# CityU-AIM-Group/SCAN

Measured on AMD Instinct MI355X. Metric: train images/sec (whole node), VGG16 C2F 1024x2048, higher is better.
Workload: dtype f32 (fp32 storage, fp32 multiply, fp32 accumulate -- the reference's arithmetic; the convolutions run it on the bf16 matrix cores as bf16x6: every fp32 operand cut into 3 bf16 pieces = all 24 significand bits, 6 bf16 MFMAs per product)

## Files before the change

### scan_amd/csrc/capi.cpp

```cpp
#include <stdarg.h>
#include <stdio.h>
#include <string.h>

#include "../../include/scan_hip.h"

static thread_local char g_err[512] = "";

extern "C" void scan_set_error(const char* fmt, ...) {
  va_list ap;
  va_start(ap, fmt);
  vsnprintf(g_err, sizeof(g_err), fmt, ap);
  va_end(ap);
}

extern "C" const char* scan_last_error(void) { return g_err; }
extern "C" int scan_abi_version(void) { return 1; }

extern int g_scan_conv_bn256;
extern int g_scan_conv_v2;
extern int g_scan_conv_wg1024;
extern int g_scan_conv_w8;
extern int g_scan_conv_tpb3;
extern int g_scan_conv_bn64_th16;
extern int g_scan_conv_glds;
extern int g_scan_conv1x1;
extern int g_scan_conv_wino;
extern int g_scan_wgrad_v6;
extern int g_scan_wgrad_prio;
extern int g_scan_wgrad_tile;
extern int g_scan_wgrad_wgs;
extern int g_scan_wgrad_wino;
extern int g_scan_gconv_mfma;
extern int g_scan_dbscan_bf16x3;
extern int g_scan_reduce_blocks;

struct Knob {
  const char* key;
  int* slot;
  int dflt;
};
static Knob* knob_table(int* count) {
  static Knob knobs[] = {
      {"conv_bn256", &g_scan_conv_bn256, 0},   {"conv_v2", &g_scan_conv_v2, 0},         {"conv_wg1024", &g_scan_conv_wg1024, 0},
      {"conv_w8", &g_scan_conv_w8, 0},         {"conv_tpb3", &g_scan_conv_tpb3, 0},     {"conv_bn64_th16", &g_scan_conv_bn64_th16, 0},
      {"conv_glds", &g_scan_conv_glds, 0},     {"wgrad_v6", &g_scan_wgrad_v6, 0},       {"wgrad_prio", &g_scan_wgrad_prio, 0},
      {"wgrad_tile", &g_scan_wgrad_tile, 0},   {"wgrad_wgs", &g_scan_wgrad_wgs, 0},     {"gconv_mfma", &g_scan_gconv_mfma, 0},
      {"dbscan_bf16x3", &g_scan_dbscan_bf16x3, 0}, {"reduce_blocks", &g_scan_reduce_blocks, 0}, {"conv1x1", &g_scan_conv1x1, 0},
      {"conv_wino", &g_scan_conv_wino, 0},     {"wgrad_wino", &g_scan_wgrad_wino, 0},
  };
  static bool init = false;
  if (!init) {
    for (auto& k : knobs) k.dflt = *k.slot;
    init = true;
  }
  *count = (int)(sizeof(knobs) / sizeof(knobs[0]));
  return knobs;
}
static Knob* find_knob(const char* key) {
  int n = 0;
  Knob* t = knob_table(&n);
  if (key == nullptr) return nullptr;
  for (int i = 0; i < n; ++i)
    if (strcmp(key, t[i].key) == 0) return &t[i];
  return nullptr;
}

extern "C" int scan_tune(const char* key, int value) {
  Knob* k = find_knob(key);
  if (k == nullptr) return SCAN_TUNE_UNKNOWN;
  const int old = *k->slot;
  *k->slot = value;
  return old;
}

extern "C" int scan_tune_get(const char* key) {
  const Knob* k = find_knob(key);
  return k == nullptr ? SCAN_TUNE_UNKNOWN : *k->slot;
}

extern "C" int scan_tune_default(const char* key) {
  const Knob* k = find_knob(key);
  return k == nullptr ? SCAN_TUNE_UNKNOWN : k->dflt;
}

extern "C" const char* scan_tune_key(int index) {
  int n = 0;
  const Knob* t = knob_table(&n);
  return (index >= 0 && index < n) ? t[index].key : nullptr;
}
```

### scan_amd/csrc/conv_fwd.hip

```cpp
#include "conv_split.h"

#define V2_TW 16
#ifndef SCAN_CONV_MID
#define SCAN_CONV_MID 0
#endif
#ifndef SCAN_CONV_PFA
#define SCAN_CONV_PFA 1
#endif
#define V2_CK 32

struct TileTab2 {
  int tile_off[SCAN_MAX_LEVELS + 1];
  int tiles_x[SCAN_MAX_LEVELS];
  int tiles_y[SCAN_MAX_LEVELS];
};

__device__ __forceinline__ int swz(int idx) { return (idx >> 1) & 2; }
__device__ __forceinline__ int wsw(int t, int r) { return ((t >> 1) & 2) ^ (r & 1); }

template <int K>
__device__ __forceinline__ const __bf16* pick_plane(const __bf16* w0, const __bf16* w1, const __bf16* w2) {
  if constexpr (K == 0)
    return w0;
  else if constexpr (K == 1)
    return w1;
  else
    return w2;
}
template <int I, int NT, int PL, int NPL>
__device__ __forceinline__ const __bf16* slot_plane(int tid, const __bf16* w0, const __bf16* w1, const __bf16* w2) {
  constexpr int lo = (NT * I) / PL, hi = (NT * I + NT - 1) / PL;
  constexpr int lo_c = lo < NPL ? lo : NPL - 1, hi_c = hi < NPL ? hi : NPL - 1;
  static_assert(hi - lo <= 1, "a thread's slot spans at most two planes");
  if constexpr (lo_c == hi_c)
    return pick_plane<lo_c>(w0, w1, w2);
  else
    return (tid + NT * I) / PL == lo ? pick_plane<lo_c>(w0, w1, w2) : pick_plane<hi_c>(w0, w1, w2);
}
template <int NT, int PL, int NPL>
__device__ __forceinline__ const __bf16* slot_plane_i(int i, int tid, const __bf16* w0, const __bf16* w1, const __bf16* w2) {
  return i == 0   ? slot_plane<0, NT, PL, NPL>(tid, w0, w1, w2)
         : i == 1 ? slot_plane<1, NT, PL, NPL>(tid, w0, w1, w2)
         : i == 2 ? slot_plane<2, NT, PL, NPL>(tid, w0, w1, w2)
         : i == 3 ? slot_plane<3, NT, PL, NPL>(tid, w0, w1, w2)
         : i == 4 ? slot_plane<4, NT, PL, NPL>(tid, w0, w1, w2)
                  : slot_plane<5, NT, PL, NPL>(tid, w0, w1, w2);
}

template <int NP, int TM>
__device__ __forceinline__ void mma_pieces(const bf16x8 (&w)[NP], const bf16x8 (&p)[NP][TM], f32x4v (&acc)[TM]) {
#pragma unroll
  for (int s = NP - 1; s >= 0; --s)
#pragma unroll
    for (int i = 0; i <= s; ++i)
#pragma unroll
      for (int tm = 0; tm < TM; ++tm) acc[tm] = __builtin_amdgcn_mfma_f32_16x16x32_bf16(w[i], p[s - i][tm], acc[tm], 0, 0, 0);
}

template <int NP, int BN, int TH, int NT, int KS, int TPB = 1, bool GL = false, bool WINO = false>
__global__ __launch_bounds__(NT, NT == 1024 ? 4 : 2) void conv_split_kernel(
    const float* __restrict__ src, scan_pyramid_t d, int Cs, const __bf16* __restrict__ w0, const __bf16* __restrict__ w1,
    const __bf16* __restrict__ w2, int Csw, const float* __restrict__ bias, const float* __restrict__ mask,
    float* __restrict__ dst, int Nout, int Ns, int relu, TileTab2 tt, int n_tiles, scan_pyramid_t sd, int map,
    double* __restrict__ gn_ws) {
  constexpr int HALO = KS / 2, NTAPS = KS * KS;
  constexpr int PH = TH + 2 * HALO;
  constexpr int PWK = WINO ? 32 : V2_TW + 2 * HALO;
  constexpr int NPATCH = PH * PWK;
  constexpr int WTAPS = WINO ? 12 : NTAPS;
  constexpr int WAVES = NT / 64;
  constexpr int WN_WAVES = BN >= 128 ? 2 : 1;
  constexpr int WM_WAVES = WAVES / WN_WAVES;
  constexpr int TM = TH / WM_WAVES;
  constexpr int TN = BN / (16 * WN_WAVES);
  constexpr int TMW = WINO ? TM / 2 : TM;
  constexpr int ASLOTS = WINO ? (PH * 64 + NT - 1) / NT : (NPATCH * 8 + NT - 1) / NT;
  constexpr int AK = WINO ? 4 : 1;
  constexpr int BSLOTS = BN * 4 * NP;
  constexpr int BSEG = (BSLOTS + NT - 1) / NT;
  constexpr int NGRP = WTAPS / TPB;
  static_assert(NP == 2 || NP == 3, "two or three pieces per operand");
  static_assert(TM * WM_WAVES == TH && (TM % 2) == 0, "tile rows must split evenly (and pair up for the fused pool)");
  static_assert(NTAPS % TPB == 0, "taps per barrier must divide the tap count");
  static_assert(BSLOTS % 64 == 0, "a wave's 64 weight segments lie in one plane (and past the end only as a whole wave)");
  static_assert(!WINO || (GL && KS == 3 && TPB == 1 && NP == 3 && TM % 2 == 0), "Winograd: three pieces, 3x3, LDS-DMA weights");

  extern __shared__ __align__(16) unsigned char smem_raw[];
  __bf16* As = reinterpret_cast<__bf16*>(smem_raw);
  __bf16* Bs = As + NP * NPATCH * 32;

  const int tid = threadIdx.x, lane = tid & 63, wid = tid >> 6;
  const int bid = xcd_remap(blockIdx.x, gridDim.x);
  const int n_tile = bid % n_tiles;
  const int tile = bid / n_tiles;
  int lvl = 0;
#pragma unroll
  for (int i = 1; i < SCAN_MAX_LEVELS; ++i)
    if (i < d.n_levels && tile >= tt.tile_off[i]) lvl = i;
  const int H = d.h[lvl], W = d.w[lvl];
  int t = tile - tt.tile_off[lvl];
  const int per_img = tt.tiles_x[lvl] * tt.tiles_y[lvl];
  const int img = t / per_img;
  t -= img * per_img;
  const int ty0 = (t / tt.tiles_x[lvl]) * TH, tx0 = (t % tt.tiles_x[lvl]) * V2_TW;
  const int64_t rowbase = d.row_off[lvl] + (int64_t)img * H * W;
  const int n0 = n_tile * BN;
  const int nchunks = (Cs + V2_CK - 1) / V2_CK;

  constexpr unsigned BAD = 0x80000000u;
  unsigned voff[ASLOTS];
  unsigned vok = 0;
  const int c_tail = Cs - (nchunks - 1) * V2_CK;
  const bool tail_bad = 4 * (tid & 7) >= c_tail;
  __amdgpu_buffer_rsrc_t a_src;
  {
    const bool mapped = KS == 1 && map != 0;
    const int Hs = mapped ? sd.h[lvl] : H, Ws = mapped ? sd.w[lvl] : W;
    int64_t base_row;
    if (!mapped)
      base_row = rowbase + (int64_t)(ty0 - HALO) * W + (tx0 - HALO);
    else if (map == 1)
      base_row = sd.row_off[lvl] + ((int64_t)img * Hs + 2 * ty0) * Ws + 2 * tx0;
    else
      base_row = sd.row_off[lvl] + ((int64_t)img * Hs + (ty0 >> 1)) * Ws + (tx0 >> 1);
    a_src = uniform_rsrc_b(src + base_row * Cs, 0x7ffffff0);
    if constexpr (WINO) {
#pragma unroll
      for (int i = 0; i < ASLOTS; ++i) {
        const int slot = tid + NT * i;
        const int c4 = slot & 7, t = (slot >> 3) & 7, py = slot >> 6;
        voff[i] = (unsigned)(((py * W + 2 * t) * Cs + 4 * c4) * 4);
#pragma unroll
        for (int k = 0; k < 4; ++k) {
          const int y = ty0 - HALO + py, x = tx0 - HALO + 2 * t + k;
          if ((slot < PH * 64) && y >= 0 && y < H && x >= 0 && x < W) vok |= 1u << (4 * i + k);
        }
      }
    } else {
#pragma unroll
      for (int i = 0; i < ASLOTS; ++i) {
        const int slot = tid + NT * i;
        const int q = slot >> 3, c4 = slot & 7;
        const int py = q / PWK, px = q - py * PWK;
        const int y = ty0 - HALO + py, x = tx0 - HALO + px;
        bool ok = (slot < NPATCH * 8) && y >= 0 && y < H && x >= 0 && x < W;
        int pix = py * W + px;
        if (mapped) {
          if (map == 1) {
            ok = ok && 2 * y < Hs && 2 * x < Ws;
            pix = 2 * py * Ws + 2 * px;
          } else {
            ok = ok && ((y | x) & 1) == 0 && (y >> 1) < Hs && (x >> 1) < Ws;
            pix = (py >> 1) * Ws + (px >> 1);
          }
        }
        voff[i] = ok ? (unsigned)((pix * Cs + 4 * c4) * 4) : BAD;
      }
    }
  }
  float4 ra[ASLOTS][AK];
  auto load_a = [&](int cc) {
    const int soff = cc * (V2_CK * 4);
    const bool kill = tail_bad && cc == nchunks - 1;
#pragma unroll
    for (int i = 0; i < ASLOTS; ++i)
#pragma unroll
      for (int k = 0; k < AK; ++k) {
        const unsigned off = !WINO ? voff[i] : ((vok >> (4 * i + k)) & 1) ? voff[i] + (unsigned)(k * Cs * 4) : BAD;
        ra[i][k] = __builtin_bit_cast(float4, __builtin_amdgcn_raw_buffer_load_b128(a_src, (int)(kill ? BAD : off), soff, 0));
      }
  };
  auto store_a = [&]() {
    if constexpr (WINO) {
#pragma unroll
      for (int i = 0; i < ASLOTS; ++i) {
        const int slot = tid + NT * i;
        if (slot < PH * 64) {
          const int c4 = slot & 7, t = (slot >> 3) & 7, py = slot >> 6;
          const float4 d0 = ra[i][0], d1 = ra[i][1], d2 = ra[i][2], d3 = ra[i][3];
          const float4 u[4] = {make_float4(d0.x - d2.x, d0.y - d2.y, d0.z - d2.z, d0.w - d2.w),
                               make_float4(d1.x + d2.x, d1.y + d2.y, d1.z + d2.z, d1.w + d2.w),
                               make_float4(d2.x - d1.x, d2.y - d1.y, d2.z - d1.z, d2.w - d1.w),
                               make_float4(d1.x - d3.x, d1.y - d3.y, d1.z - d3.z, d1.w - d3.w)};
          const int sl = (((c4 >> 1) ^ wsw(t, py)) << 3) + ((c4 & 1) << 2);
#pragma unroll
          for (int j = 0; j < 4; ++j) {
            bf16x4 pc[NP];
            split4_np<NP>(u[j], pc);
            const int off = (py * PWK + j * 8 + t) * 32 + sl;
#pragma unroll
            for (int p = 0; p < NP; ++p) *reinterpret_cast<bf16x4*>(As + p * NPATCH * 32 + off) = pc[p];
          }
        }
      }
      return;
    }
#pragma unroll
    for (int i = 0; i < ASLOTS; ++i) {
      const int slot = tid + NT * i;
      if (slot < NPATCH * 8) {
        const int q = slot >> 3, c4 = slot & 7;
        const int px = q % PWK;
        bf16x4 pc[NP];
        split4_np<NP>(ra[i][0], pc);
        const int off = q * 32 + (((c4 >> 1) ^ swz(px)) << 3) + ((c4 & 1) << 2);
#pragma unroll
        for (int p = 0; p < NP; ++p) *reinterpret_cast<bf16x4*>(As + p * NPATCH * 32 + off) = pc[p];
      }
    }
  };
  uint4 rb[TPB][BSEG];
  auto load_b = [&](int cc, int grp) {
#pragma unroll
    for (int tt = 0; tt < TPB; ++tt) {
      const int tap = grp * TPB + tt;
#pragma unroll
      for (int i = 0; i < BSEG; ++i) {
        const int slot = tid + NT * i;
        const int plane = slot / (BN * 4);
        const int rem = slot - plane * BN * 4;
        const int row = rem >> 2, seg = rem & 3;
        const int o = n0 + row, c = cc * V2_CK + 8 * seg;
        const __bf16* base = slot_plane_i<NT, BN * 4, NP>(i, tid, w0, w1, w2);
        rb[tt][i] = (slot < BSLOTS && o < Nout && c < Csw)
                        ? *reinterpret_cast<const uint4*>(base + ((int64_t)o * NTAPS + tap) * Csw + c)
                        : make_uint4(0u, 0u, 0u, 0u);
      }
    }
  };
  auto store_b = [&](int buf) {
#pragma unroll
    for (int tt = 0; tt < TPB; ++tt) {
#pragma unroll
      for (int i = 0; i < BSEG; ++i) {
        const int slot = tid + NT * i;
        const int plane = slot / (BN * 4);
        const int rem = slot - plane * BN * 4;
        const int row = rem >> 2, seg = rem & 3;
        if (slot < BSLOTS)
          *reinterpret_cast<uint4*>(Bs + (((buf * TPB + tt) * NP + plane) * BN + row) * 32 + ((seg ^ swz(row)) << 3)) = rb[tt][i];
      }
    }
  };

  static_assert(!GL || BSEG <= 6, "the LDS-DMA path keeps at most six descriptors");
  unsigned boff[BSEG];
#pragma unroll
  for (int i = 0; i < BSEG; ++i) {
    const int slot = tid + NT * i;
    const int plane = slot / (BN * 4);
    const int rem = slot - plane * BN * 4;
    const int row = rem >> 2, seg = (rem & 3) ^ swz(row);
    boff[i] = (unsigned)((((n0 + row) * WTAPS) * Csw + 8 * seg) * 2);
  }
  const int plane_bytes = Nout * WTAPS * Csw * 2;
  auto plane_rsrc = [&](int i) { return uniform_rsrc_b(slot_plane_i<NT, BN * 4, NP>(i, tid, w0, w1, w2), plane_bytes); };
  const __amdgpu_buffer_rsrc_t b_src0 = plane_rsrc(0), b_src1 = plane_rsrc(1), b_src2 = plane_rsrc(2),
                               b_src3 = plane_rsrc(3), b_src4 = plane_rsrc(4), b_src5 = plane_rsrc(5);
  auto issue_b = [&](int cc, int grp, int buf) {
#pragma unroll
    for (int tt = 0; tt < TPB; ++tt) {
      const int tap = grp * TPB + tt;
      const int soff = (tap * Csw + cc * V2_CK) * 2;
#pragma unroll
      for (int i = 0; i < BSEG; ++i) {
        const int slot = tid + NT * i;
        if (BSEG * NT != BSLOTS && slot - lane >= BSLOTS) continue;
        const int plane = slot / (BN * 4);
        const int rem = slot - plane * BN * 4;
        __bf16* dst_l = Bs + (((buf * TPB + tt) * NP + plane) * BN) * 32 + (rem - lane) * 8;
        __builtin_amdgcn_raw_ptr_buffer_load_lds(
            i == 0 ? b_src0 : i == 1 ? b_src1 : i == 2 ? b_src2 : i == 3 ? b_src3 : i == 4 ? b_src4 : b_src5, (lds_ptr_t)dst_l,
            16, (int)boff[i], soff, 0, 0);
      }
    }
  };

  const int wm = wid / WN_WAVES, wn = wid % WN_WAVES;
  const int lr = lane & 15, kg = lane >> 4;
  const int w_row0 = wn * 16 * TN + lr;
  const int w_off = w_row0 * 32 + ((kg ^ swz(w_row0)) << 3);

  f32x4v acc[TN][TM];
#pragma unroll
  for (int b = 0; b < TN; ++b)
#pragma unroll
    for (int a = 0; a < TM; ++a) acc[b][a] = f32x4v{0.f, 0.f, 0.f, 0.f};
  f32x4v wacc[WINO ? 4 : 1][WINO ? TN : 1][TMW];
#pragma unroll
  for (int j = 0; j < (WINO ? 4 : 1); ++j)
#pragma unroll
    for (int b = 0; b < (WINO ? TN : 1); ++b)
#pragma unroll
      for (int a = 0; a < TMW; ++a) wacc[j][b][a] = f32x4v{0.f, 0.f, 0.f, 0.f};

  auto patch_off = [&](int tap) {
    const int ky = tap / KS, kx = tap - KS * ky;
    const int pxs = lr + kx;
    return ((wm * TM + ky) * PWK + pxs) * 32 + ((kg ^ swz(pxs)) << 3);
  };
  auto read_patch = [&](int tap, bf16x8 (&pf)[NP][TM]) {
    const int p_off = patch_off(tap);
#pragma unroll
    for (int p = 0; p < NP; ++p)
#pragma unroll
      for (int tm = 0; tm < TM; ++tm)
        pf[p][tm] = *reinterpret_cast<const bf16x8*>(As + p * NPATCH * 32 + p_off + tm * PWK * 32);
  };
  auto read_w = [&](const __bf16* bt, int tn, bf16x8 (&wf)[NP]) {
#pragma unroll
    for (int p = 0; p < NP; ++p) wf[p] = *reinterpret_cast<const bf16x8*>(bt + p * BN * 32 + tn * 16 * 32);
  };
  auto taps_mma = [&](int grp, int buf, auto&& mid) {
#pragma unroll
    for (int tt = 0; tt < TPB; ++tt) {
      const int tap = grp * TPB + tt;
      const __bf16* bt = Bs + ((buf * TPB + tt) * NP) * BN * 32 + w_off;
      bf16x8 pf[NP][TM];
      read_patch(tap, pf);
#pragma unroll
      for (int tn = 0; tn < TN; ++tn) {
        bf16x8 wf[NP];
        read_w(bt, tn, wf);
        mma_pieces<NP, TM>(wf, pf, acc[tn]);
#ifdef SCAN_EXP_MID_STAGGER
        if (tt == 0 && tn == ((wid >= WAVES / 2 && TN >= 8) ? SCAN_EXP_MID_STAGGER : SCAN_CONV_MID)) {
#else
        if (tt == 0 && tn == SCAN_CONV_MID) {
#endif
          __builtin_amdgcn_sched_barrier(0);
          mid();
          __builtin_amdgcn_sched_barrier(0);
        }
      }
    }
  };
  auto no_mid = []() {};

  constexpr bool PFA = GL && NT == 512 && TPB == 1 && NP == 2 && SCAN_CONV_PFA;
  bf16x8 npf[NP][TM];
  auto taps_mma_pf = [&](int grp, int buf, auto&& mid) {
    if constexpr (PFA) {
      const __bf16* bt = Bs + (buf * NP) * BN * 32 + w_off;
      if (grp == 0) read_patch(0, npf);
#pragma unroll
      for (int tn = 0; tn < TN - 1; ++tn) {
        bf16x8 wf[NP];
        read_w(bt, tn, wf);
        mma_pieces<NP, TM>(wf, npf, acc[tn]);
        if (tn == SCAN_CONV_MID) {
          __builtin_amdgcn_sched_barrier(0);
          mid();
          __builtin_amdgcn_sched_barrier(0);
        }
      }
      {
        constexpr int tn = TN - 1;
        bf16x8 wf[NP];
        read_w(bt, tn, wf);
        const bool more = grp < NGRP - 1;
        const int p_off = patch_off(more ? grp + 1 : grp);
#pragma unroll
        for (int tm = 0; tm < TM; ++tm) {
          acc[tn][tm] = __builtin_amdgcn_mfma_f32_16x16x32_bf16(wf[0], npf[1][tm], acc[tn][tm], 0, 0, 0);
          acc[tn][tm] = __builtin_amdgcn_mfma_f32_16x16x32_bf16(wf[1], npf[0][tm], acc[tn][tm], 0, 0, 0);
          acc[tn][tm] = __builtin_amdgcn_mfma_f32_16x16x32_bf16(wf[0], npf[0][tm], acc[tn][tm], 0, 0, 0);
          npf[0][tm] = *reinterpret_cast<const bf16x8*>(As + p_off + tm * PWK * 32);
          npf[1][tm] = *reinterpret_cast<const bf16x8*>(As + NPATCH * 32 + p_off + tm * PWK * 32);
        }
      }
    }
  };

  auto wino_mma = [&](int j, int ky, int buf, f32x4v (&aj)[WINO ? TN : 1][TMW], auto&& mid) {
    const __bf16* bt = Bs + (buf * NP) * BN * 32 + w_off;
    const int prow = wm * TM + (lr >> 3) + ky, t = lr & 7;
    const int p_off = (prow * PWK + j * 8 + t) * 32 + ((kg ^ wsw(t, prow)) << 3);
    bf16x8 pf[NP][TMW];
#pragma unroll
    for (int p = 0; p < NP; ++p)
#pragma unroll
      for (int tm = 0; tm < TMW; ++tm)
        pf[p][tm] = *reinterpret_cast<const bf16x8*>(As + p * NPATCH * 32 + p_off + tm * 2 * PWK * 32);
#pragma unroll
    for (int tn = 0; tn < TN; ++tn) {
      bf16x8 wf[NP];
      read_w(bt, tn, wf);
      mma_pieces<NP, TMW>(wf, pf, aj[tn]);
      if (tn == (SCAN_CONV_MID >= 0 ? SCAN_CONV_MID : 0)) {
        __builtin_amdgcn_sched_barrier(0);
        mid();
        __builtin_amdgcn_sched_barrier(0);
      }
    }
  };

  load_a(0);
  if constexpr (WINO) {
    issue_b(0, 0, 0);
    for (int cc = 0; cc < nchunks; ++cc) {
      __syncthreads();
      store_a();
      auto comp = [&](int j, f32x4v (&aj)[WINO ? TN : 1][TMW]) {
#pragma unroll 1
        for (int ky = 0; ky < 3; ++ky) {
          const int grp = j * 3 + ky, buf = grp & 1;
          asm volatile("s_waitcnt vmcnt(0)" ::: "memory");
          __syncthreads();
          auto feed = [&]() {
            if (grp < NGRP - 1)
              issue_b(cc, grp + 1, buf ^ 1);
            else if (cc + 1 < nchunks)
              issue_b(cc + 1, 0, buf ^ 1);
            if (grp == NGRP - 2 && cc + 1 < nchunks) load_a(cc + 1);
          };
          wino_mma(j, ky, buf, aj, feed);
        }
      };
      comp(0, wacc[0]);
      comp(1, wacc[WINO ? 1 : 0]);
      comp(2, wacc[WINO ? 2 : 0]);
      comp(3, wacc[WINO ? 3 : 0]);
    }
  } else if constexpr (GL) {
    issue_b(0, 0, 0);
    for (int cc = 0; cc < nchunks; ++cc) {
      __syncthreads();
#ifdef SCAN_EXP_FWD_NOFEED
      if (cc == 0 || !(SCAN_EXP_FWD_NOFEED & 2))
#endif
      store_a();
      if (NGRP == 1 && cc + 1 < nchunks) load_a(cc + 1);
#pragma unroll 1
      for (int grp = 0; grp < NGRP; ++grp) {
        const int buf = (cc * NGRP + grp) & 1;
        asm volatile("s_waitcnt vmcnt(0)" ::: "memory");
        __syncthreads();
        auto feed = [&]() {
#ifdef SCAN_EXP_FWD_NOFEED
          if ((SCAN_EXP_FWD_NOFEED & 1) && !(SCAN_EXP_FWD_NOFEED & 2)) {
            if (NGRP > 1 && grp == NGRP - 2 && cc + 1 < nchunks) load_a(cc + 1);
            return;
          }
          if ((SCAN_EXP_FWD_NOFEED & 3) == 3) return;
#endif
          if (grp < NGRP - 1)
            issue_b(cc, grp + 1, buf ^ 1);
          else if (cc + 1 < nchunks)
            issue_b(cc + 1, 0, buf ^ 1);
          if (NGRP > 1 && grp == NGRP - 2 && cc + 1 < nchunks) load_a(cc + 1);
        };
        if constexpr (PFA) {
          taps_mma_pf(grp, buf, feed);
        } else if (SCAN_CONV_MID >= 0) {
          taps_mma(grp, buf, feed);
        } else {
          feed();
          taps_mma(grp, buf, no_mid);
        }
      }
    }
  } else {
    load_b(0, 0);
    for (int cc = 0; cc < nchunks; ++cc) {
      __syncthreads();
      store_a();
      if (cc + 1 < nchunks) load_a(cc + 1);
#pragma unroll 1
      for (int grp = 0; grp < NGRP; ++grp) {
        const int buf = (cc * NGRP + grp) & 1;
        store_b(buf);
        if (grp < NGRP - 1)
          load_b(cc, grp + 1);
        else if (cc + 1 < nchunks)
          load_b(cc + 1, 0);
        __syncthreads();
        taps_mma(grp, buf, no_mid);
      }
    }
  }

  const int x = tx0 + lr;
  double* gn_red = reinterpret_cast<double*>(smem_raw);
  if (gn_ws != nullptr) __syncthreads();
#pragma unroll
  for (int tn = 0; tn < TN; ++tn) {
    const int o4 = n0 + wn * 16 * TN + tn * 16 + 4 * kg;
    float4 bv = make_float4(0.f, 0.f, 0.f, 0.f);
    if (bias != nullptr) {
      bv.x = o4 + 0 < Nout ? bias[o4 + 0] : 0.f;
      bv.y = o4 + 1 < Nout ? bias[o4 + 1] : 0.f;
      bv.z = o4 + 2 < Nout ? bias[o4 + 2] : 0.f;
      bv.w = o4 + 3 < Nout ? bias[o4 + 3] : 0.f;
    }
    if constexpr (WINO) {
      const int xw = tx0 + 2 * (lr & 7);
      if (relu & 2) {
#pragma unroll
        for (int tm = 0; tm < TMW; ++tm) {
          const int y = ty0 + wm * TM + 2 * tm + (lr >> 3);
          const f32x4v m0 = wacc[0][tn][tm], m1 = wacc[WINO ? 1 : 0][tn][tm], m2 = wacc[WINO ? 2 : 0][tn][tm],
                       m3 = wacc[WINO ? 3 : 0][tn][tm];
          const f32x4v y0 = m0 + (m1 + m2), y1 = (m1 - m2) - m3;
          float v[4];
#pragma unroll
          for (int r = 0; r < 4; ++r) {
            const float m = fmaxf(y0[r], y1[r]);
            v[r] = fmaxf(m, __shfl_xor(m, 8, 64));
          }
          if ((lr >> 3) == 0 && y < H && xw < W && o4 < Nout) {
            const int Hp = H >> 1, Wp = W >> 1;
            float4 o = make_float4(v[0] + bv.x, v[1] + bv.y, v[2] + bv.z, v[3] + bv.w);
            if (relu & 1) {
              o.x = fmaxf(o.x, 0.f);
              o.y = fmaxf(o.y, 0.f);
              o.z = fmaxf(o.z, 0.f);
              o.w = fmaxf(o.w, 0.f);
            }
            *reinterpret_cast<float4*>(dst + ((int64_t)img * Hp * Wp + (int64_t)(y >> 1) * Wp + (xw >> 1)) * Ns + o4) = o;
          }
        }
        continue;
      }
      float4 mk[TMW][2];
      if (mask != nullptr) {
#pragma unroll
        for (int tm = 0; tm < TMW; ++tm) {
          const int y = ty0 + wm * TM + 2 * tm + (lr >> 3);
#pragma unroll
          for (int e = 0; e < 2; ++e) {
            const bool ok = y < H && xw + e < W && o4 < Nout;
            mk[tm][e] = ok ? *reinterpret_cast<const float4*>(mask + (rowbase + (int64_t)y * W + xw + e) * Ns + o4)
                           : make_float4(0.f, 0.f, 0.f, 0.f);
          }
        }
      }
      double ds = 0.0, dq = 0.0;
#pragma unroll
      for (int tm = 0; tm < TMW; ++tm) {
        const int y = ty0 + wm * TM + 2 * tm + (lr >> 3);
        const f32x4v m0 = wacc[0][tn][tm], m1 = wacc[WINO ? 1 : 0][tn][tm], m2 = wacc[WINO ? 2 : 0][tn][tm],
                     m3 = wacc[WINO ? 3 : 0][tn][tm];
        const f32x4v yv[2] = {m0 + (m1 + m2), (m1 - m2) - m3};
#pragma unroll
        for (int e = 0; e < 2; ++e) {
          if (y < H && xw + e < W && o4 < Nout) {
            float4 o = make_float4(yv[e][0] + bv.x, yv[e][1] + bv.y, yv[e][2] + bv.z, yv[e][3] + bv.w);
            if (relu & 1) {
              o.x = fmaxf(o.x, 0.f);
              o.y = fmaxf(o.y, 0.f);
              o.z = fmaxf(o.z, 0.f);
              o.w = fmaxf(o.w, 0.f);
            }
            if (mask != nullptr) {
              o.x = (mk[tm][e].x > 0.f) ? o.x : 0.f;
              o.y = (mk[tm][e].y > 0.f) ? o.y : 0.f;
              o.z = (mk[tm][e].z > 0.f) ? o.z : 0.f;
              o.w = (mk[tm][e].w > 0.f) ? o.w : 0.f;
            }
            *reinterpret_cast<float4*>(dst + (rowbase + (int64_t)y * W + xw + e) * Ns + o4) = o;
            ds += (double)((o.x + o.y) + (o.z + o.w));
            dq += (double)((o.x * o.x + o.y * o.y) + (o.z * o.z + o.w * o.w));
          }
        }
      }
      if (gn_ws != nullptr) {
#pragma unroll
        for (int sh = 1; sh <= 16; sh <<= 1) {
          ds += __shfl_xor(ds, sh, 64);
          dq += __shfl_xor(dq, sh, 64);
        }
        if (lr == 0 && (kg & 1) == 0) {
          double* r = gn_red + (wm * (BN / 8) + ((o4 - n0) >> 3)) * 2;
          r[0] = ds;
          r[1] = dq;
        }
      }
      continue;
    }
    if (relu & 2) {
      const int Hp = H >> 1, Wp = W >> 1;
#pragma unroll
      for (int tm = 0; tm < TM; tm += 2) {
        const int y = ty0 + wm * TM + tm;
        float v[4];
#pragma unroll
        for (int r = 0; r < 4; ++r) {
          const float m = fmaxf(acc[tn][tm][r], acc[tn][tm + 1][r]);
          v[r] = fmaxf(m, __shfl_xor(m, 1, 64));
        }
        if ((lr & 1) == 0 && y < H && x < W && o4 < Nout) {
          float4 o = make_float4(v[0] + bv.x, v[1] + bv.y, v[2] + bv.z, v[3] + bv.w);
          if (relu & 1) {
            o.x = fmaxf(o.x, 0.f);
            o.y = fmaxf(o.y, 0.f);
            o.z = fmaxf(o.z, 0.f);
            o.w = fmaxf(o.w, 0.f);
          }
          *reinterpret_cast<float4*>(dst + ((int64_t)img * Hp * Wp + (int64_t)(y >> 1) * Wp + (x >> 1)) * Ns + o4) = o;
        }
      }
      continue;
    }
    float4 mk[TM];
    if (mask != nullptr) {
#pragma unroll
      for (int tm = 0; tm < TM; ++tm) {
        const int y = ty0 + wm * TM + tm;
        const bool ok = y < H && x < W && o4 < Nout;
        mk[tm] = ok ? *reinterpret_cast<const float4*>(mask + (rowbase + (int64_t)y * W + x) * Ns + o4)
                    : make_float4(0.f, 0.f, 0.f, 0.f);
      }
    }
    double ds = 0.0, dq = 0.0;
#pragma unroll
    for (int tm = 0; tm < TM; ++tm) {
      const int y = ty0 + wm * TM + tm;
      if (y < H && x < W && o4 < Nout) {
        float4 o = make_float4(acc[tn][tm][0] + bv.x, acc[tn][tm][1] + bv.y, acc[tn][tm][2] + bv.z,
                               acc[tn][tm][3] + bv.w);
        if (relu & 1) {
          o.x = fmaxf(o.x, 0.f);
          o.y = fmaxf(o.y, 0.f);
          o.z = fmaxf(o.z, 0.f);
          o.w = fmaxf(o.w, 0.f);
        }
        if (mask != nullptr) {
          o.x = (mk[tm].x > 0.f) ? o.x : 0.f;
          o.y = (mk[tm].y > 0.f) ? o.y : 0.f;
          o.z = (mk[tm].z > 0.f) ? o.z : 0.f;
          o.w = (mk[tm].w > 0.f) ? o.w : 0.f;
        }
#ifdef SCAN_EXP_FWD_NOSTORE
        if (o.x == 1.2345e30f)
#endif
        *reinterpret_cast<float4*>(dst + (rowbase + (int64_t)y * W + x) * Ns + o4) = o;
        ds += (double)((o.x + o.y) + (o.z + o.w));
        dq += (double)((o.x * o.x + o.y * o.y) + (o.z * o.z + o.w * o.w));
      }
    }
    if (gn_ws != nullptr) {
#pragma unroll
      for (int sh = 1; sh <= 16; sh <<= 1) {
        ds += __shfl_xor(ds, sh, 64);
        dq += __shfl_xor(dq, sh, 64);
      }
      if (lr == 0 && (kg & 1) == 0) {
        double* r = gn_red + (wm * (BN / 8) + ((o4 - n0) >> 3)) * 2;
        r[0] = ds;
        r[1] = dq;
      }
    }
  }
  if (gn_ws != nullptr) {
    __syncthreads();
    if (tid < BN / 8 * 2) {
      const int g = n0 / 8 + (tid >> 1);
      double v = 0.0;
#pragma unroll
      for (int w = 0; w < WM_WAVES; ++w) v += gn_red[w * (BN / 8) * 2 + tid];
      if (g * 8 < Nout) atomicAdd(&gn_ws[((int64_t)(lvl * d.n_images + img) * 32 + g) * 2 + (tid & 1)], v);
    }
  }
}

static void make_tiles_v2(const scan_pyramid_t* d, TileTab2* tt, int TH) {
  tt->tile_off[0] = 0;
  for (int l = 0; l < SCAN_MAX_LEVELS; ++l) {
    if (l < d->n_levels) {
      tt->tiles_x[l] = (d->w[l] + V2_TW - 1) / V2_TW;
      tt->tiles_y[l] = (d->h[l] + TH - 1) / TH;
      tt->tile_off[l + 1] = tt->tile_off[l] + d->n_images * tt->tiles_x[l] * tt->tiles_y[l];
    } else {
      tt->tiles_x[l] = tt->tiles_y[l] = 1;
      tt->tile_off[l + 1] = tt->tile_off[l];
    }
  }
}

struct ConvArgs {
  const float* x;
  const scan_pyramid_t* od;
  const scan_pyramid_t* sd;
  int32_t Cs;
  const __bf16* w[3];
  int32_t Csw;
  const float* bias;
  const float* mask;
  float* y;
  int32_t Nout, Ns, relu, map;
  hipStream_t st;
  double* gn_ws;
};

template <int NP, int BN, int TH, int NT, int KS, int TPB = 1, bool GL = false, bool WINO = false>
static void launch_v2(const ConvArgs& a) {
  constexpr int HALO = KS / 2;
  TileTab2 tt;
  make_tiles_v2(a.od, &tt, TH);
  const int tiles = tt.tile_off[a.od->n_levels];
  const int n_tiles = (a.Nout + BN - 1) / BN;
  constexpr int PWK = WINO ? 32 : V2_TW + 2 * HALO;
  constexpr size_t sh = (size_t)(NP * (TH + 2 * HALO) * PWK * 32 + 2 * NP * TPB * BN * 32) * sizeof(__bf16);
  static_assert(sh <= 160 * 1024, "LDS: 160 KB per CU");
  static bool done = false;
  if (!done) {
    hipFuncSetAttribute(reinterpret_cast<const void*>(conv_split_kernel<NP, BN, TH, NT, KS, TPB, GL, WINO>),
                        hipFuncAttributeMaxDynamicSharedMemorySize, (int)sh);
    done = true;
  }
  hipLaunchKernelGGL((conv_split_kernel<NP, BN, TH, NT, KS, TPB, GL, WINO>), dim3(tiles * n_tiles), dim3(NT), sh, a.st, a.x, *a.od,
                     a.Cs, a.w[0], a.w[1], a.w[2], a.Csw, a.bias, a.mask, a.y, a.Nout, a.Ns, a.relu, tt, n_tiles, *a.sd,
                     a.map, a.gn_ws);
}

int g_scan_conv_bn256 = 2;
int g_scan_conv_wg1024 = 1;
int g_scan_conv_w8 = 1;
int g_scan_conv_tpb3 = 1;
int g_scan_conv_glds = 1;
int g_scan_conv_bn64_th16 = 2;
static int v2_instance(const scan_pyramid_t* od, int32_t Nout) {
  if (Nout <= 64) return 64;
  TileTab2 tt;
  make_tiles_v2(od, &tt, 16);
  const int64_t tiles = tt.tile_off[od->n_levels];
  if (g_scan_conv_bn256 == 1 && Nout % 256 == 0 && tiles * (Nout / 256) >= 512) return 256;
  if (g_scan_conv_bn256 == 2 && Nout % 256 == 0) {
    const int64_t r256 = (tiles * (Nout / 256) + 255) / 256 * 2, r128 = (tiles * (Nout / 128) + 255) / 256;
    if (r256 * 97 <= r128 * 100) return 256;
  }
  return 128;
}

int conv3x3_split_launch(int np, const float* x, const scan_pyramid_t* d, int32_t Cs, const void* w0, const void* w1,
                         const void* w2, int32_t Csw, const float* bias, const float* mask, float* y, int32_t Nout,
                         int32_t Ns, int32_t relu, void* stream, double* gn_ws) {
  ConvArgs a{x, d, d, Cs, {reinterpret_cast<const __bf16*>(w0), reinterpret_cast<const __bf16*>(w1),
                           reinterpret_cast<const __bf16*>(w2)}, Csw, bias, mask, y, Nout, Ns, relu, 0, as_stream(stream), gn_ws};
  const bool whole = g_scan_conv_glds && Csw % 32 == 0;
  const bool th16 = g_scan_conv_bn64_th16 && d->n_levels == 1 && d->h[0] % 16 == 0 && d->w[0] % 16 == 0;
  if (np == 3) {
    switch (v2_instance(d, Nout)) {
      case 64:
        if (whole && th16 && g_scan_conv_bn64_th16 == 2 && d->h[0] % 32 == 0)
          launch_v2<3, 64, 32, 512, 3, 1, true>(a);
        else if (whole && th16)
          launch_v2<3, 64, 16, 512, 3, 1, true>(a);
        else if (whole)
          launch_v2<3, 64, 8, 256, 3, 1, true>(a);
        else if (th16)
          launch_v2<3, 64, 16, 512, 3>(a);
        else
          launch_v2<3, 64, 8, 256, 3>(a);
        break;
      case 256:
        if (whole)
          launch_v2<3, 256, 16, 512, 3, 1, true>(a);
        else
          launch_v2<3, 256, 16, 512, 3>(a);
        break;
      default:
        if (whole)
          launch_v2<3, 128, 16, 512, 3, 1, true>(a);
        else
          launch_v2<3, 128, 16, 512, 3>(a);
        break;
    }
    SCAN_LAUNCH_CHECK("conv3x3_bf16x6");
    return 0;
  }
  switch (v2_instance(d, Nout)) {
    case 64:
      if (th16)
        launch_v2<2, 64, 16, 256, 3>(a);
      else if (g_scan_conv_tpb3 & 2)
        launch_v2<2, 64, 8, 256, 3, 3>(a);
      else
        launch_v2<2, 64, 8, 256, 3>(a);
      break;
    case 256:
      if (g_scan_conv_w8 && g_scan_conv_wg1024 == 1 && whole)
        launch_v2<2, 256, 16, 512, 3, 1, true>(a);
      else if ((g_scan_conv_wg1024 == 1 || (g_scan_conv_wg1024 == 2 && d->n_levels > 1)) && whole)
        launch_v2<2, 256, 16, 1024, 3, 1, true>(a);
      else if (g_scan_conv_wg1024 == 1 || (g_scan_conv_wg1024 == 2 && d->n_levels > 1))
        launch_v2<2, 256, 16, 1024, 3>(a);
      else
        launch_v2<2, 256, 16, 512, 3>(a);
      break;
    default:
      if (g_scan_conv_wg1024 == 1 && (g_scan_conv_tpb3 & 1) && whole && Nout % 128 == 0)
        launch_v2<2, 128, 16, 1024, 3, 3, true>(a);
      else if (g_scan_conv_wg1024 == 1 && (g_scan_conv_tpb3 & 1))
        launch_v2<2, 128, 16, 1024, 3, 3>(a);
      else if (g_scan_conv_wg1024 == 1 && whole && Nout % 128 == 0)
        launch_v2<2, 128, 16, 1024, 3, 1, true>(a);
      else if (g_scan_conv_wg1024 == 1)
        launch_v2<2, 128, 16, 1024, 3>(a);
      else if (g_scan_conv_tpb3 & 1)
        launch_v2<2, 128, 16, 512, 3, 3>(a);
      else
        launch_v2<2, 128, 16, 512, 3>(a);
      break;
  }
  SCAN_LAUNCH_CHECK("conv3x3_bf16x3");
  return 0;
}

int g_scan_conv_wino = 1;
extern "C" int scan_conv3x3_bf16x6_wino(int32_t Nout, int32_t Csw) { return g_scan_conv_wino && Nout > 64 && Csw % 32 == 0 ? 1 : 0; }

int conv3x3_wino_launch(const float* x, const scan_pyramid_t* d, int32_t Cs, const void* w0, const void* w1, const void* w2,
                        int32_t Csw, const float* bias, const float* mask, float* y, int32_t Nout, int32_t Ns, int32_t relu,
                        void* stream, double* gn_ws) {
  SCAN_CHECK_ARG(Nout > 64 && Csw % 32 == 0, "conv3x3_wino_bf16x6: needs Nout > 64 and Csw %% 32 == 0 (Nout=%d Csw=%d)", Nout, Csw);
  ConvArgs a{x, d, d, Cs, {reinterpret_cast<const __bf16*>(w0), reinterpret_cast<const __bf16*>(w1),
                           reinterpret_cast<const __bf16*>(w2)}, Csw, bias, mask, y, Nout, Ns, relu, 0, as_stream(stream), gn_ws};
  launch_v2<3, 128, 16, 512, 3, 1, true, true>(a);
  SCAN_LAUNCH_CHECK("conv3x3_wino_bf16x6");
  return 0;
}

static int conv1x1_instance3(const scan_pyramid_t* yd, int32_t Nout, int32_t Csw);
int g_scan_conv1x1 = 3;
static int conv1x1_instance3(const scan_pyramid_t* yd, int32_t Nout, int32_t Csw) {
  if (Nout <= 64) return 64;
  if (!((g_scan_conv1x1 & 1) && Csw % 32 == 0)) return 128;
  if ((g_scan_conv1x1 & 2) && Nout % 256 == 0) {
    TileTab2 tt;
    make_tiles_v2(yd, &tt, 16);
    const int64_t tiles = tt.tile_off[yd->n_levels];
    const int64_t r256 = (tiles * (Nout / 256) + 255) / 256 * 2, r128 = (tiles * (Nout / 128) + 255) / 256;
    if (r256 * 97 <= r128 * 100) return 1256;
  }
  return 1128;
}
extern "C" int scan_conv1x1_bf16x6_instance(const scan_pyramid_t* yd, int32_t Nout, int32_t Csw) {
  return yd ? conv1x1_instance3(yd, Nout, Csw) : -1;
}

int conv1x1_split_launch(int np, const float* x, const scan_pyramid_t* xd, int32_t Cs, const void* w0, const void* w1,
                         const void* w2, int32_t Csw, const float* bias, const float* mask, float* y,
                         const scan_pyramid_t* yd, int32_t Nout, int32_t Ns, int32_t relu, int32_t map, void* stream) {
  ConvArgs a{x, yd, xd, Cs, {reinterpret_cast<const __bf16*>(w0), reinterpret_cast<const __bf16*>(w1),
                             reinterpret_cast<const __bf16*>(w2)}, Csw, bias, mask, y, Nout, Ns, relu, map, as_stream(stream), nullptr};
  const int inst = np == 3 ? conv1x1_instance3(yd, Nout, Csw) : (Nout <= 64 ? 64 : 128);
  const bool wide = inst == 1256, gl = inst >= 1000;
  if (np == 3) {
    if (Nout <= 64)
      launch_v2<3, 64, 8, 256, 1>(a);
    else if (wide)
      launch_v2<3, 256, 16, 512, 1, 1, true>(a);
    else if (gl)
      launch_v2<3, 128, 16, 512, 1, 1, true>(a);
    else
      launch_v2<3, 128, 16, 512, 1>(a);
  } else {
    if (Nout <= 64)
      launch_v2<2, 64, 8, 256, 1>(a);
    else
      launch_v2<2, 128, 16, 512, 1>(a);
  }
  SCAN_LAUNCH_CHECK("conv1x1_split");
  return 0;
}

extern "C" int scan_conv3x3_bf16x3_instance(const scan_pyramid_t* d, int32_t Nout) {
  if (!d) return -1;
  const int bn = v2_instance(d, Nout);
  if (bn == 256 && g_scan_conv_w8 && g_scan_conv_wg1024 == 1 && g_scan_conv_glds) return 2256;
  if (bn == 256 && (g_scan_conv_wg1024 == 1 || (g_scan_conv_wg1024 == 2 && d->n_levels > 1))) return 1256;
  if (bn == 128 && g_scan_conv_wg1024 == 1) return 1128;
  return bn;
}

extern "C" int scan_conv3x3_bf16x6_instance(const scan_pyramid_t* d, int32_t Nout) {
  if (!d) return -1;
  const int bn = v2_instance(d, Nout);
  if (bn == 64 && g_scan_conv_bn64_th16 && d->n_levels == 1 && d->h[0] % 16 == 0 && d->w[0] % 16 == 0)
    return (g_scan_conv_bn64_th16 == 2 && d->h[0] % 32 == 0) ? 2064 : 1064;
  return bn;
}
```

Measured before the change: 24.32.

## Add two-taps-per-barrier Winograd forward conv variant with half-width patch staging

Adds a TPB=2 instance of the Winograd bf16x6 forward convolution, now the default. Each barrier interval processes two tap groups, halving the synchronisations per chunk. The input patch is staged in two halves with half the LDS width, and weight fragments are double-buffered in registers so reads overlap the MFMAs. It also adds a compiler-opaque lane remap in the epilogue and a different input-load addressing. The cost is more code complexity, plus extra register pressure that may limit occupancy.

Measured after the change: 25.05 (median of 6 runs). 3.0% higher.

```diff
diff --git a/scan_amd/csrc/capi.cpp b/scan_amd/csrc/capi.cpp
--- a/scan_amd/csrc/capi.cpp
+++ b/scan_amd/csrc/capi.cpp
@@ -25,6 +25,7 @@
 extern int g_scan_conv_glds;
 extern int g_scan_conv1x1;
 extern int g_scan_conv_wino;
+extern int g_scan_wino_tpb;
 extern int g_scan_wgrad_v6;
 extern int g_scan_wgrad_prio;
 extern int g_scan_wgrad_tile;
@@ -46,7 +47,7 @@
       {"conv_glds", &g_scan_conv_glds, 0},     {"wgrad_v6", &g_scan_wgrad_v6, 0},       {"wgrad_prio", &g_scan_wgrad_prio, 0},
       {"wgrad_tile", &g_scan_wgrad_tile, 0},   {"wgrad_wgs", &g_scan_wgrad_wgs, 0},     {"gconv_mfma", &g_scan_gconv_mfma, 0},
       {"dbscan_bf16x3", &g_scan_dbscan_bf16x3, 0}, {"reduce_blocks", &g_scan_reduce_blocks, 0}, {"conv1x1", &g_scan_conv1x1, 0},
-      {"conv_wino", &g_scan_conv_wino, 0},     {"wgrad_wino", &g_scan_wgrad_wino, 0},
+      {"conv_wino", &g_scan_conv_wino, 0},     {"wgrad_wino", &g_scan_wgrad_wino, 0},   {"wino_tpb", &g_scan_wino_tpb, 0},
   };
   static bool init = false;
   if (!init) {
diff --git a/scan_amd/csrc/conv_fwd.hip b/scan_amd/csrc/conv_fwd.hip
--- a/scan_amd/csrc/conv_fwd.hip
+++ b/scan_amd/csrc/conv_fwd.hip
@@ -17,6 +17,11 @@
 
 __device__ __forceinline__ int swz(int idx) { return (idx >> 1) & 2; }
 __device__ __forceinline__ int wsw(int t, int r) { return ((t >> 1) & 2) ^ (r & 1); }
+
+template <int V>
+struct IntC {
+  static constexpr int value = V;
+};
 
 template <int K>
 __device__ __forceinline__ const __bf16* pick_plane(const __bf16* w0, const __bf16* w1, const __bf16* w2) {
@@ -65,7 +70,8 @@
     double* __restrict__ gn_ws) {
   constexpr int HALO = KS / 2, NTAPS = KS * KS;
   constexpr int PH = TH + 2 * HALO;
-  constexpr int PWK = WINO ? 32 : V2_TW + 2 * HALO;
+  constexpr int WJ = WINO ? (TPB == 2 ? 2 : 4) : 1;
+  constexpr int PWK = WINO ? WJ * 8 : V2_TW + 2 * HALO;
   constexpr int NPATCH = PH * PWK;
   constexpr int WTAPS = WINO ? 12 : NTAPS;
   constexpr int WAVES = NT / 64;
@@ -81,9 +87,9 @@
   constexpr int NGRP = WTAPS / TPB;
   static_assert(NP == 2 || NP == 3, "two or three pieces per operand");
   static_assert(TM * WM_WAVES == TH && (TM % 2) == 0, "tile rows must split evenly (and pair up for the fused pool)");
-  static_assert(NTAPS % TPB == 0, "taps per barrier must divide the tap count");
+  static_assert(WTAPS % TPB == 0, "taps per barrier must divide the tap count");
   static_assert(BSLOTS % 64 == 0, "a wave's 64 weight segments lie in one plane (and past the end only as a whole wave)");
-  static_assert(!WINO || (GL && KS == 3 && TPB == 1 && NP == 3 && TM % 2 == 0), "Winograd: three pieces, 3x3, LDS-DMA weights");
+  static_assert(!WINO || (GL && KS == 3 && (TPB == 1 || TPB == 2) && NP == 3 && TM % 2 == 0), "Winograd: three pieces, 3x3, LDS-DMA weights");
 
   extern __shared__ __align__(16) unsigned char smem_raw[];
   __bf16* As = reinterpret_cast<__bf16*>(smem_raw);
@@ -162,6 +168,19 @@
   auto load_a = [&](int cc) {
     const int soff = cc * (V2_CK * 4);
     const bool kill = tail_bad && cc == nchunks - 1;
+    if constexpr (WINO && TPB == 2) {
+      unsigned vk = vok;
+      asm volatile("" : "+v"(vk));
+#pragma unroll
+      for (int i = 0; i < ASLOTS; ++i)
+#pragma unroll
+        for (int k = 0; k < AK; ++k) {
+          const bool ok = ((vk >> (4 * i + k)) & 1) && !kill;
+          ra[i][k] = __builtin_bit_cast(float4, __builtin_amdgcn_raw_buffer_load_b128(a_src, (int)(ok ? voff[0] : BAD),
+                                                                                      soff + (i * (NT / 64) * W + k) * Cs * 4, 0));
+        }
+      return;
+    }
 #pragma unroll
     for (int i = 0; i < ASLOTS; ++i)
 #pragma unroll
@@ -170,8 +189,9 @@
         ra[i][k] = __builtin_bit_cast(float4, __builtin_amdgcn_raw_buffer_load_b128(a_src, (int)(kill ? BAD : off), soff, 0));
       }
   };
-  auto store_a = [&]() {
+  auto store_a = [&](auto half_c) {
     if constexpr (WINO) {
+      constexpr int half = decltype(half_c)::value;
 #pragma unroll
       for (int i = 0; i < ASLOTS; ++i) {
         const int slot = tid + NT * i;
@@ -184,9 +204,9 @@
                                make_float4(d1.x - d3.x, d1.y - d3.y, d1.z - d3.z, d1.w - d3.w)};
           const int sl = (((c4 >> 1) ^ wsw(t, py)) << 3) + ((c4 & 1) << 2);
 #pragma unroll
-          for (int j = 0; j < 4; ++j) {
+          for (int j = 0; j < WJ; ++j) {
             bf16x4 pc[NP];
-            split4_np<NP>(u[j], pc);
+            split4_np<NP>(u[WJ == 4 ? j : 2 * half + j], pc);
             const int off = (py * PWK + j * 8 + t) * 32 + sl;
 #pragma unroll
             for (int p = 0; p < NP; ++p) *reinterpret_cast<bf16x4*>(As + p * NPATCH * 32 + off) = pc[p];
@@ -372,8 +392,8 @@
     }
   };
 
-  auto wino_mma = [&](int j, int ky, int buf, f32x4v (&aj)[WINO ? TN : 1][TMW], auto&& mid) {
-    const __bf16* bt = Bs + (buf * NP) * BN * 32 + w_off;
+  auto wino_mma = [&](int j, int ky, int buf, f32x4v (&aj)[WINO ? TN : 1][TMW], auto&& mid, int tt = 0, bool with_mid = true) {
+    const __bf16* bt = Bs + ((buf * TPB + tt) * NP) * BN * 32 + w_off;
     const int prow = wm * TM + (lr >> 3) + ky, t = lr & 7;
     const int p_off = (prow * PWK + j * 8 + t) * 32 + ((kg ^ wsw(t, prow)) << 3);
     bf16x8 pf[NP][TMW];
@@ -382,12 +402,28 @@
 #pragma unroll
       for (int tm = 0; tm < TMW; ++tm)
         pf[p][tm] = *reinterpret_cast<const bf16x8*>(As + p * NPATCH * 32 + p_off + tm * 2 * PWK * 32);
+    if constexpr (TPB == 2) {
+      bf16x8 wf2[2][NP];
+      read_w(bt, 0, wf2[0]);
+#pragma unroll
+      for (int tn = 0; tn < TN; ++tn) {
+        if (tn + 1 < TN) read_w(bt, tn + 1, wf2[(tn + 1) & 1]);
+        __builtin_amdgcn_sched_barrier(0);
+        mma_pieces<NP, TMW>(wf2[tn & 1], pf, aj[tn]);
+        __builtin_amdgcn_sched_barrier(0);
+        if (with_mid && tn == 0) {
+          mid();
+          __builtin_amdgcn_sched_barrier(0);
+        }
+      }
+      return;
+    }
 #pragma unroll
     for (int tn = 0; tn < TN; ++tn) {
       bf16x8 wf[NP];
       read_w(bt, tn, wf);
       mma_pieces<NP, TMW>(wf, pf, aj[tn]);
-      if (tn == (SCAN_CONV_MID >= 0 ? SCAN_CONV_MID : 0)) {
+      if (with_mid && tn == (SCAN_CONV_MID >= 0 ? SCAN_CONV_MID : 0)) {
         __builtin_amdgcn_sched_barrier(0);
         mid();
         __builtin_amdgcn_sched_barrier(0);
@@ -396,11 +432,39 @@
   };
 
   load_a(0);
-  if constexpr (WINO) {
+  if constexpr (WINO && TPB == 2) {
+    issue_b(0, 0, 0);
+    for (int cc = 0; cc < nchunks; ++cc) {
+      auto ivl = [&](auto g_c, int j0, int ky0, f32x4v (&a0)[WINO ? TN : 1][TMW], int j1, int ky1, f32x4v (&a1)[WINO ? TN : 1][TMW]) {
+        constexpr int g = decltype(g_c)::value, buf = g & 1;
+        asm volatile("s_waitcnt vmcnt(0)" ::: "memory");
+        __syncthreads();
+        auto feed = [&]() {
+          if (g < NGRP - 1)
+            issue_b(cc, g + 1, buf ^ 1);
+          else if (cc + 1 < nchunks)
+            issue_b(cc + 1, 0, buf ^ 1);
+          if (g == NGRP / 2 && cc + 1 < nchunks) load_a(cc + 1);
+        };
+        wino_mma(j0, ky0, buf, a0, feed, 0, true);
+        wino_mma(j1, ky1, buf, a1, no_mid, 1, false);
+      };
+      auto phase = [&](auto half_c, f32x4v (&a0)[WINO ? TN : 1][TMW], f32x4v (&a1)[WINO ? TN : 1][TMW]) {
+        __syncthreads();
+        constexpr int half = decltype(half_c)::value;
+        store_a(half_c);
+        ivl(IntC<3 * half + 0>{}, 0, 0, a0, 0, 1, a0);
+        ivl(IntC<3 * half + 1>{}, 0, 2, a0, 1, 0, a1);
+        ivl(IntC<3 * half + 2>{}, 1, 1, a1, 1, 2, a1);
+      };
+      phase(IntC<0>{}, wacc[0], wacc[WINO ? 1 : 0]);
+      phase(IntC<1>{}, wacc[WINO ? 2 : 0], wacc[WINO ? 3 : 0]);
+    }
+  } else if constexpr (WINO) {
     issue_b(0, 0, 0);
     for (int cc = 0; cc < nchunks; ++cc) {
       __syncthreads();
-      store_a();
+      store_a(IntC<0>{});
       auto comp = [&](int j, f32x4v (&aj)[WINO ? TN : 1][TMW]) {
 #pragma unroll 1
         for (int ky = 0; ky < 3; ++ky) {
@@ -429,7 +493,7 @@
 #ifdef SCAN_EXP_FWD_NOFEED
       if (cc == 0 || !(SCAN_EXP_FWD_NOFEED & 2))
 #endif
-      store_a();
+      store_a(IntC<0>{});
       if (NGRP == 1 && cc + 1 < nchunks) load_a(cc + 1);
 #pragma unroll 1
       for (int grp = 0; grp < NGRP; ++grp) {
@@ -464,7 +528,7 @@
     load_b(0, 0);
     for (int cc = 0; cc < nchunks; ++cc) {
       __syncthreads();
-      store_a();
+      store_a(IntC<0>{});
       if (cc + 1 < nchunks) load_a(cc + 1);
 #pragma unroll 1
       for (int grp = 0; grp < NGRP; ++grp) {
@@ -480,12 +544,18 @@
     }
   }
 
-  const int x = tx0 + lr;
+  constexpr bool RELANE = WINO && TPB == 2;
+  int tid2 = tid;
+  if constexpr (RELANE) asm volatile("" : "+v"(tid2));
+  const int etid = RELANE ? tid2 : tid;
+  const int ewm = RELANE ? (tid2 >> 6) / WN_WAVES : wm, ewn = RELANE ? (tid2 >> 6) % WN_WAVES : wn;
+  const int elr = RELANE ? tid2 & 15 : lr, ekg = RELANE ? (tid2 & 63) >> 4 : kg;
+  const int x = tx0 + elr;
   double* gn_red = reinterpret_cast<double*>(smem_raw);
   if (gn_ws != nullptr) __syncthreads();
 #pragma unroll
   for (int tn = 0; tn < TN; ++tn) {
-    const int o4 = n0 + wn * 16 * TN + tn * 16 + 4 * kg;
+    const int o4 = n0 + ewn * 16 * TN + tn * 16 + 4 * ekg;
     float4 bv = make_float4(0.f, 0.f, 0.f, 0.f);
     if (bias != nullptr) {
       bv.x = o4 + 0 < Nout ? bias[o4 + 0] : 0.f;
@@ -494,11 +564,11 @@
       bv.w = o4 + 3 < Nout ? bias[o4 + 3] : 0.f;
     }
     if constexpr (WINO) {
-      const int xw = tx0 + 2 * (lr & 7);
+      const int xw = tx0 + 2 * (elr & 7);
       if (relu & 2) {
 #pragma unroll
         for (int tm = 0; tm < TMW; ++tm) {
-          const int y = ty0 + wm * TM + 2 * tm + (lr >> 3);
+          const int y = ty0 + ewm * TM + 2 * tm + (elr >> 3);
           const f32x4v m0 = wacc[0][tn][tm], m1 = wacc[WINO ? 1 : 0][tn][tm], m2 = wacc[WINO ? 2 : 0][tn][tm],
                        m3 = wacc[WINO ? 3 : 0][tn][tm];
           const f32x4v y0 = m0 + (m1 + m2), y1 = (m1 - m2) - m3;
@@ -508,7 +578,7 @@
             const float m = fmaxf(y0[r], y1[r]);
             v[r] = fmaxf(m, __shfl_xor(m, 8, 64));
           }
-          if ((lr >> 3) == 0 && y < H && xw < W && o4 < Nout) {
+          if ((elr >> 3) == 0 && y < H && xw < W && o4 < Nout) {
             const int Hp = H >> 1, Wp = W >> 1;
             float4 o = make_float4(v[0] + bv.x, v[1] + bv.y, v[2] + bv.z, v[3] + bv.w);
             if (relu & 1) {
@@ -526,7 +596,7 @@
       if (mask != nullptr) {
 #pragma unroll
         for (int tm = 0; tm < TMW; ++tm) {
-          const int y = ty0 + wm * TM + 2 * tm + (lr >> 3);
+          const int y = ty0 + ewm * TM + 2 * tm + (elr >> 3);
 #pragma unroll
           for (int e = 0; e < 2; ++e) {
             const bool ok = y < H && xw + e < W && o4 < Nout;
@@ -538,7 +608,7 @@
       double ds = 0.0, dq = 0.0;
 #pragma unroll
       for (int tm = 0; tm < TMW; ++tm) {
-        const int y = ty0 + wm * TM + 2 * tm + (lr >> 3);
+        const int y = ty0 + ewm * TM + 2 * tm + (elr >> 3);
         const f32x4v m0 = wacc[0][tn][tm], m1 = wacc[WINO ? 1 : 0][tn][tm], m2 = wacc[WINO ? 2 : 0][tn][tm],
                      m3 = wacc[WINO ? 3 : 0][tn][tm];
         const f32x4v yv[2] = {m0 + (m1 + m2), (m1 - m2) - m3};
@@ -570,8 +640,8 @@
           ds += __shfl_xor(ds, sh, 64);
           dq += __shfl_xor(dq, sh, 64);
         }
-        if (lr == 0 && (kg & 1) == 0) {
-          double* r = gn_red + (wm * (BN / 8) + ((o4 - n0) >> 3)) * 2;
+        if (elr == 0 && (ekg & 1) == 0) {
+          double* r = gn_red + (ewm * (BN / 8) + ((o4 - n0) >> 3)) * 2;
           r[0] = ds;
           r[1] = dq;
         }
@@ -582,14 +652,14 @@
       const int Hp = H >> 1, Wp = W >> 1;
 #pragma unroll
       for (int tm = 0; tm < TM; tm += 2) {
-        const int y = ty0 + wm * TM + tm;
+        const int y = ty0 + ewm * TM + tm;
         float v[4];
 #pragma unroll
         for (int r = 0; r < 4; ++r) {
           const float m = fmaxf(acc[tn][tm][r], acc[tn][tm + 1][r]);
           v[r] = fmaxf(m, __shfl_xor(m, 1, 64));
         }
-        if ((lr & 1) == 0 && y < H && x < W && o4 < Nout) {
+        if ((elr & 1) == 0 && y < H && x < W && o4 < Nout) {
           float4 o = make_float4(v[0] + bv.x, v[1] + bv.y, v[2] + bv.z, v[3] + bv.w);
           if (relu & 1) {
             o.x = fmaxf(o.x, 0.f);
@@ -606,7 +676,7 @@
     if (mask != nullptr) {
 #pragma unroll
       for (int tm = 0; tm < TM; ++tm) {
-        const int y = ty0 + wm * TM + tm;
+        const int y = ty0 + ewm * TM + tm;
         const bool ok = y < H && x < W && o4 < Nout;
         mk[tm] = ok ? *reinterpret_cast<const float4*>(mask + (rowbase + (int64_t)y * W + x) * Ns + o4)
                     : make_float4(0.f, 0.f, 0.f, 0.f);
@@ -615,7 +685,7 @@
     double ds = 0.0, dq = 0.0;
 #pragma unroll
     for (int tm = 0; tm < TM; ++tm) {
-      const int y = ty0 + wm * TM + tm;
+      const int y = ty0 + ewm * TM + tm;
       if (y < H && x < W && o4 < Nout) {
         float4 o = make_float4(acc[tn][tm][0] + bv.x, acc[tn][tm][1] + bv.y, acc[tn][tm][2] + bv.z,
                                acc[tn][tm][3] + bv.w);
@@ -645,8 +715,8 @@
         ds += __shfl_xor(ds, sh, 64);
         dq += __shfl_xor(dq, sh, 64);
       }
-      if (lr == 0 && (kg & 1) == 0) {
-        double* r = gn_red + (wm * (BN / 8) + ((o4 - n0) >> 3)) * 2;
+      if (elr == 0 && (ekg & 1) == 0) {
+        double* r = gn_red + (ewm * (BN / 8) + ((o4 - n0) >> 3)) * 2;
         r[0] = ds;
         r[1] = dq;
       }
@@ -654,12 +724,12 @@
   }
   if (gn_ws != nullptr) {
     __syncthreads();
-    if (tid < BN / 8 * 2) {
-      const int g = n0 / 8 + (tid >> 1);
+    if (etid < BN / 8 * 2) {
+      const int g = n0 / 8 + (etid >> 1);
       double v = 0.0;
 #pragma unroll
-      for (int w = 0; w < WM_WAVES; ++w) v += gn_red[w * (BN / 8) * 2 + tid];
-      if (g * 8 < Nout) atomicAdd(&gn_ws[((int64_t)(lvl * d.n_images + img) * 32 + g) * 2 + (tid & 1)], v);
+      for (int w = 0; w < WM_WAVES; ++w) v += gn_red[w * (BN / 8) * 2 + etid];
+      if (g * 8 < Nout) atomicAdd(&gn_ws[((int64_t)(lvl * d.n_images + img) * 32 + g) * 2 + (etid & 1)], v);
     }
   }
 }
@@ -700,7 +770,7 @@
   make_tiles_v2(a.od, &tt, TH);
   const int tiles = tt.tile_off[a.od->n_levels];
   const int n_tiles = (a.Nout + BN - 1) / BN;
-  constexpr int PWK = WINO ? 32 : V2_TW + 2 * HALO;
+  constexpr int PWK = WINO ? (TPB == 2 ? 16 : 32) : V2_TW + 2 * HALO;
   constexpr size_t sh = (size_t)(NP * (TH + 2 * HALO) * PWK * 32 + 2 * NP * TPB * BN * 32) * sizeof(__bf16);
   static_assert(sh <= 160 * 1024, "LDS: 160 KB per CU");
   static bool done = false;
@@ -809,6 +879,7 @@
 }
 
 int g_scan_conv_wino = 1;
+int g_scan_wino_tpb = 2;
 extern "C" int scan_conv3x3_bf16x6_wino(int32_t Nout, int32_t Csw) { return g_scan_conv_wino && Nout > 64 && Csw % 32 == 0 ? 1 : 0; }
 
 int conv3x3_wino_launch(const float* x, const scan_pyramid_t* d, int32_t Cs, const void* w0, const void* w1, const void* w2,
@@ -817,7 +888,10 @@
   SCAN_CHECK_ARG(Nout > 64 && Csw % 32 == 0, "conv3x3_wino_bf16x6: needs Nout > 64 and Csw %% 32 == 0 (Nout=%d Csw=%d)", Nout, Csw);
   ConvArgs a{x, d, d, Cs, {reinterpret_cast<const __bf16*>(w0), reinterpret_cast<const __bf16*>(w1),
                            reinterpret_cast<const __bf16*>(w2)}, Csw, bias, mask, y, Nout, Ns, relu, 0, as_stream(stream), gn_ws};
-  launch_v2<3, 128, 16, 512, 3, 1, true, true>(a);
+  if (g_scan_wino_tpb == 2)
+    launch_v2<3, 128, 16, 512, 3, 2, true, true>(a);
+  else
+    launch_v2<3, 128, 16, 512, 3, 1, true, true>(a);
   SCAN_LAUNCH_CHECK("conv3x3_wino_bf16x6");
   return 0;
 }
```
